# oadrian/GPUFluidSimulator

Measured on AMD Instinct MI355X. Metric: particle-steps/sec, higher is better.
Workload: dtype f32; 1 GPU; dam-break C3: 256x256x256 = 16777216 particles, grid 512^3, box 32.0, dt 5e-7, jittered lattice, FLOWING: timed after 6000 run-up steps on the device (+5 warm-up); particles=16777216, parallelism=1 GPU, whole domain, state=flow, runup_steps=6000

## Files before the change

gpufluidsimulator_amd/capi.py:

```python
from __future__ import annotations

import ctypes as C
import functools
import os

import numpy as np

HERE = os.path.dirname(os.path.abspath(__file__))
LIB_PATH = os.environ.get("SPH_HIP_LIB", os.path.join(HERE, "libsph_hip.so"))

PHASES = ("z-index", "sort", "b-grid", "dens", "force", "collision", "integrate")
HALO_RECORD_FLOATS = 8


class SphError(RuntimeError):
    pass


EXCHANGE_FN = C.CFUNCTYPE(C.c_int, C.c_void_p, C.c_int, C.c_void_p, C.c_size_t, C.c_void_p, C.c_size_t, C.c_void_p, C.c_size_t,
                          C.c_void_p, C.c_size_t, C.c_void_p)


class Transport(C.Structure):
    _fields_ = [("self", C.c_void_p), ("exchange", EXCHANGE_FN), ("host_buffers", C.c_int),
# ... 238 lines not shown
    "sph_get_order": (C.c_int, [_P, _P]),
    "sph_get_cell_range": (C.c_int, [_P, _U32, C.POINTER(_U32), C.POINTER(_U32)]),
    "sph_get_cells": (C.c_int, [_P, _U32, _P, _P, _P]),
    "sph_cell_key": (_U32, [_P, _U32, _U32, _U32]),
    "sph_hash": (C.c_int, [_P]),
    "sph_sort": (C.c_int, [_P]),
    "sph_build_cells": (C.c_int, [_P]),
    "sph_density": (C.c_int, [_P]),
    "sph_force": (C.c_int, [_P]),
    "sph_collide": (C.c_int, [_P]),
    "sph_integrate": (C.c_int, [_P, C.c_float]),
    "sph_step": (C.c_int, [_P, C.c_float, _U32]),
    "sph_step_phased": (C.c_int, [_P, C.c_float, _U32]),
    "sph_force_collide_integrate": (C.c_int, [_P, C.c_float]),
    "sph_timing_enable": (C.c_int, [_P, C.c_int]),
    "sph_timing_get": (C.c_int, [_P, C.POINTER(C.c_float), C.POINTER(_U32)]),
    "sph_timing_reset": (C.c_int, [_P]),
    "sph_last_sort_skipped": (C.c_int, [_P]),
    "sph_sort_stats": (C.c_int, [_P, C.POINTER(C.c_uint64), C.POINTER(C.c_uint64), C.POINTER(C.c_uint64), C.POINTER(C.c_uint32),
                                 C.POINTER(C.c_uint64)]),
    "sph_set_sort_mode": (C.c_int, [_P, C.c_int]),
    "sph_set_direct_hull": (C.c_int, [_P, C.c_uint32]),
    "sph_set_pair_small_launch": (C.c_int, [_P, C.c_uint32]),
    "sph_set_block_order": (C.c_int, [_P, C.c_int, C.c_int, C.c_uint32]),
    "sph_sort_forms": (C.c_int, [_P, C.POINTER(C.c_uint64)]),
    "sph_test_trust_mover_hint": (C.c_int, [_P]),
    "sph_memory_stats": (None, [C.POINTER(C.c_uint64)]),
    "sph_test_fail_alloc": (None, [C.c_uint32]),
    "sph_test_guard": (None, [C.c_uint32, C.c_int]),
    "sph_test_guard_check": (C.c_int, [C.POINTER(C.c_uint64)]),
    "sph_test_scan": (C.c_int, [_P, C.c_int, C.c_uint32, C.c_void_p, C.c_void_p, C.c_void_p]),
    "sph_test_lower_bounds": (C.c_int, [_P, C.c_void_p, C.c_uint32, C.c_void_p, C.c_uint32, C.c_void_p]),
    "sph_set_precision": (C.c_int, [_P, C.c_int]),
    "sph_get_precision": (C.c_int, [_P]),
    "sph_migrants_count": (C.c_int, [_P, C.POINTER(_U32)]),
    "sph_slab_counts": (C.c_int, [_P, C.POINTER(_U32)]),
    "sph_migrants_pack": (C.c_int, [_P, C.POINTER(_P), _U32]),
    "sph_migrants_append": (C.c_int, [_P, _P, _U32]),
    "sph_halo_count": (C.c_int, [_P, C.POINTER(_U32)]),
    "sph_halo_pack": (C.c_int, [_P, C.POINTER(_P), _U32]),
    "sph_halo_pack_counts": (C.c_int, [_P, C.POINTER(_P), _U32, C.POINTER(_U32)]),
    "sph_halo_unpack": (C.c_int, [_P, _P, _U32, _P, _U32]),
    "sph_halo_pack_density": (C.c_int, [_P, C.POINTER(_P), _U32]),
    "sph_halo_unpack_density": (C.c_int, [_P, _P, _P]),
    "sph_layer_histogram": (C.c_int, [_P, _P, _U32]),
    "sph_rccl_unique_id": (C.c_int, [C.c_void_p]),
# ... 668 lines not shown
        return out, total[0]

    def test_lower_bounds(self, keys, targets):
        k, t = np.ascontiguousarray(keys), np.ascontiguousarray(targets)
        assert k.ndim == 1 and t.ndim == 1 and k.dtype == np.uint32 and t.dtype == np.uint32, (k.dtype, t.dtype)
        out = np.empty(t.size, np.uint32)
        _check(self.L.sph_test_lower_bounds(self.h, k.ctypes.data, k.size, t.ctypes.data, t.size, out.ctypes.data))
        return out

    def sort_forms(self):
        out = (C.c_uint64 * 3)()
        _check(self.L.sph_sort_forms(self.h, out))
        return tuple(int(v) for v in out)

    def set_block_order(self, xcd=True, ztile=True, strip_blocks_log2=4):
        _check(self.L.sph_set_block_order(self.h, int(bool(xcd)), int(bool(ztile)), int(strip_blocks_log2)))

    def set_direct_hull(self, slots=512):
        _check(self.L.sph_set_direct_hull(self.h, int(slots) & 0xFFFFFFFF))

    def set_pair_small_launch(self, slots):
        _check(self.L.sph_set_pair_small_launch(self.h, int(slots) & 0xFFFFFFFF))

    def timing_get(self):
        ms = (C.c_float * len(PHASES))()
        steps = _U32(0)
        _check(self.L.sph_timing_get(self.h, ms, C.byref(steps)))
        return {PHASES[k]: float(ms[k]) for k in range(len(PHASES))}, int(steps.value)

    def _pair(self, fn, *a):
        cnt = (_U32 * 2)()
        _check(fn(self.h, cnt, *a))
        return int(cnt[0]), int(cnt[1])

    def slab_counts(self):
        cnt = (_U32 * 4)()
        _check(self.L.sph_slab_counts(self.h, cnt))
        return tuple(int(v) for v in cnt)

    def force_collide_integrate(self, dt): _check(self.L.sph_force_collide_integrate(self.h, float(dt)))

    def migrants_count(self): return self._pair(self.L.sph_migrants_count)
    def halo_count(self): return self._pair(self.L.sph_halo_count)

    def migrants_pack(self, buf_lo, buf_hi, capacity):
        _check(self.L.sph_migrants_pack(self.h, (_P * 2)(buf_lo, buf_hi), int(capacity)))
# ... 26 lines not shown
```

gpufluidsimulator_amd/csrc/sph_capi.hip:

```cpp
#include "sph_device.hpp"

#include <cmath>
#include <cstdarg>
#include <cstdlib>
#include <cstring>
#include <mutex>
#include <new>
#include <vector>

namespace sph {

template <class T>
__global__ __launch_bounds__(1024) void k_test_scan(const T* __restrict__ in, uint32_t n, T* __restrict__ out, T* __restrict__ total) {
    __shared__ T lds[1024 / 64];
    const T sum = scan_array_one_block<1024>(n, lds, [&](uint32_t i) { return in[i]; }, [&](uint32_t i, T before) { out[i] = before; });
    if (threadIdx.x == 0) *total = sum;
}

template <class T>
static int test_scan(sph_ctx* c, Buffers& mem, uint32_t n, const void* in, void* out, void* total) {
    T *d_in = nullptr, *d_out = nullptr, *d_total = nullptr;
    int rc;
    if ((rc = mem.alloc(&d_in, n, false)) || (rc = mem.alloc(&d_out, n, false)) || (rc = mem.alloc(&d_total, 1, false))) return rc;
    if (n) SPH_HIP(hipMemcpyAsync(d_in, in, (size_t)n * sizeof(T), hipMemcpyHostToDevice, c->stream));
// ... 215 lines not shown
    c->device = device;
    c->ghost_layers = slab ? ghost_layers : 1u;
    int rc = derive(c, p, z_lo, z_hi, slab);
    if (rc) { delete c; return rc; }
    c->cap = capacity; c->gcap = gcap; c->tot = capacity + 2 * gcap; c->slab = slab;
    c->own_off = gcap;
    c->pos_out_cap = slab ? 0 : capacity;
    Buffers& m = c->mem;
    const size_t tot = (size_t)c->tot + 256;
    rc = m.alloc(&c->posi, tot, true);
    if (!rc) rc = m.alloc(&c->velr, tot, true);
    if (!rc) rc = m.alloc(&c->posi2, tot, true);
    if (!rc) rc = m.alloc(&c->velr2, tot, true);
    if (!rc) rc = m.alloc(&c->keyS, tot, true);
    if (!rc) rc = m.alloc(&c->keyS2, tot, true);
    if (!rc) rc = m.alloc(&c->dp, tot, true);
    if (!rc) rc = m.alloc(&c->cw, tot, true);
    if (!rc) rc = m.alloc(&c->fpress, tot, false);
    if (!rc) rc = m.alloc(&c->fvisc, tot, false);
    if (!rc) rc = m.alloc(&c->dvel, tot, false);
    if (!rc) rc = m.alloc(&c->pos_out, (size_t)c->pos_out_cap, false);
    if (!rc) rc = m.alloc(&c->table.base, (size_t)c->grid.ncells + 2, true);
    if (!rc) table_init(c, c->table.base, c->grid.ncells);
    if (!rc) rc = sort_buffers_alloc(c);
    if (const char* env = getenv("SPH_BLOCK_ORDER")) {
        int x = 1, z = 1, sh = 4, zd = 1, xr = 1;
        if (sscanf(env, "%d,%d,%d,%d,%d", &x, &z, &sh, &zd, &xr) >= 1) {
            c->order_xcd = x != 0; c->order_ztile = z != 0; if (sh >= 1 && sh <= 10) c->order_strip_sh = (uint32_t)sh;
            c->order_ztile_dens = zd != 0; c->order_xrot = xr != 0;
        }
    }
    if (const char* env = getenv("SPH_PAIR_SMALL_SLOTS")) {
        unsigned long v = 0;
        if (sscanf(env, "%lu", &v) == 1) c->pair_small_slots = v > 0xFFFFFFFFul ? 0xFFFFFFFFu : (uint32_t)v;
    }
    if (const char* env = getenv("SPH_PAIR_CLAMP")) {
        int v = 1;
        if (sscanf(env, "%d", &v) == 1) c->pair_clamp = v != 0;
    }
    if (rc) { m.free_all(); delete c; return rc; }
    *out = c;
    return SPH_OK;
}

void timing_collect(sph_ctx* c) {
    for (size_t k = 0; k + 3 <= c->events.size(); k += 3) {
        hipEvent_t a = c->events[k], b = c->events[k + 1];
        int phase = (int)(intptr_t)c->events[k + 2];
        hipEventSynchronize(b);
        float ms = 0.f;
        if (hipEventElapsedTime(&ms, a, b) == hipSuccess) c->ph_ms[phase] += ms;
        hipEventDestroy(a);
        hipEventDestroy(b);
    }
    c->events.clear();
}

int step_hash(sph_ctx* c, bool ghosts_to_sort) {
    PhaseTimer t(c, SPH_PH_ZINDEX);
    const SlotRange live = live_slots(c);
    int rc = c->sort_merge && c->order_valid && table_covers(c, live.lo, live.hi) ? table_leave_to_sort(c, ghosts_to_sort)
// ... 815 lines not shown
}

int sph_set_block_order(sph_ctx* c, int xcd, int ztile, uint32_t strip_blocks_log2) {
    SPH_REQUIRE(c, SPH_E_INVALID, "null context");
    SPH_REQUIRE(strip_blocks_log2 >= 1u && strip_blocks_log2 <= 10u, SPH_E_INVALID, "strip of 2^%u blocks", strip_blocks_log2);
    c->order_xcd = xcd != 0;
    c->order_ztile = c->order_ztile_dens = ztile != 0;
    c->order_strip_sh = strip_blocks_log2;
    return SPH_OK;
}

int sph_set_direct_hull(sph_ctx* c, uint32_t slots) {
    SPH_REQUIRE(c, SPH_E_INVALID, "null context");
    c->direct_hull = slots;
    return SPH_OK;
}

int sph_set_pair_small_launch(sph_ctx* c, uint32_t slots) {
    SPH_REQUIRE(c, SPH_E_INVALID, "null context");
    c->pair_small_slots = slots;
    return SPH_OK;
}

int sph_sort_stats(sph_ctx* c, uint64_t* sorts, uint64_t* merges, uint64_t* skips, uint32_t* last_movers,
                   uint64_t* movers_total) {
    SPH_REQUIRE(c, SPH_E_INVALID, "null context");
    SPH_HIP(hipSetDevice(c->device));
    SPH_HIP(hipStreamSynchronize(c->stream));
    if (movers_total) {
        unsigned long long t = 0;
        SPH_HIP(hipMemcpy(&t, c->mm_total, sizeof(t), hipMemcpyDeviceToHost));
        *movers_total = t;
    }
    if (sorts) *sorts = c->sort_calls;
    if (merges) *merges = c->sort_merges;
    if (skips) *skips = c->sort_skips;
    if (last_movers) *last_movers = c->mm_count_host[HW_MOVERS];
    return SPH_OK;
}

void sph_memory_stats(uint64_t out[3]) {
    if (out) for (int k = 0; k < 3; k++) out[k] = g_mem_stats[k].load();
}

void sph_test_fail_alloc(uint32_t k) { g_fail_alloc.store(k); }

// ... 35 lines not shown
```

gpufluidsimulator_amd/csrc/sph_common.hpp:

```cpp
#pragma once

#include <hip/hip_runtime.h>

#include <atomic>
#include <cstdint>
#include <cstdio>
#include <cstring>
#include <string>
#include <utility>
#include <vector>

#include "../../include/sph_hip.h"

namespace sph {

constexpr int WAVE = 64;
#ifndef SPH_SORT_KPT
#define SPH_SORT_KPT 16
#endif
constexpr uint32_t SORT_TILE_KEYS = 256 * SPH_SORT_KPT;
#ifndef SPH_PAIR_SMALL_SLOTS_DEFAULT
#define SPH_PAIR_SMALL_SLOTS_DEFAULT 524288u
#endif
constexpr uint32_t MM_TILE_CHUNKS = 256;
// ... 115 lines not shown
        return SPH_OK;
    }
    static void drop(const Rec& r) {
        void* base = r.p;
        if (r.band) { guard_retire(r.p, r.bytes, r.band, r.pinned); base = (char*)r.p - r.band; }
        if (r.pinned) hipHostFree(base); else hipFree(base);
        g_mem_stats[r.pinned] -= r.bytes; g_mem_stats[2] -= 1;
    }
};

enum class TableLeft : uint8_t {
    NOTHING,
    OWNED,
    OWNED_AND_GHOSTS
};

struct CellTable {
    uint2* cells = nullptr;
    uint2* base = nullptr;
    uint32_t alloc = 0;
    uint32_t lo = 0, hi = 0;
    bool valid = false;
    TableLeft left = TableLeft::NOTHING;
};

struct MoverMarks {
    bool marked = false;
    bool scanned = false;
    uint32_t off = 0, n = 0;
    uint32_t scan_seq = 0;
    bool counted_valid = false;
};

enum HostWord : uint32_t {
    HW_MOVERS = 0,
    HW_FIRST_KEY,
    HW_LAST_KEY,
    HW_BUILD_SEQ,
    HW_COUNT_SEQ,
    HW_WORDS = 8
};

struct ObstacleBodyBlock {
    double quat[4];
    float off[3], u[3], pivot[3], omega[3];
    float rot[9], P[3];
};

struct Obstacle {
    sph_obstacle_grid grid{};
    float* phi = nullptr;
    float* brick = nullptr;
    float off[3] = {0.f, 0.f, 0.f}, vel[3] = {0.f, 0.f, 0.f};
    bool posed = false;
    float pivot[3] = {0.f, 0.f, 0.f}, omega[3] = {0.f, 0.f, 0.f};
    double quat[4] = {1.0, 0.0, 0.0, 0.0};
    bool sense = false;
    double* rows = nullptr;
    uint32_t* wmask = nullptr;
    double* load = nullptr;
    bool body = false;
    sph_obstacle_body bd{};
// ... 69 lines not shown
    float* rd_sf_normal = nullptr;
    bool rd_surface = false;
    bool rd_sf_thick_on = false;
    bool rd_solids = false;
    sph_solid_style rd_solid_style{};
    float* rd_so_depth = nullptr;
    uint32_t* rd_so_slot = nullptr;
    float* rd_so_normal = nullptr;

    uint32_t* mesh_field = nullptr;
    uint32_t* mesh_vbase = nullptr;
    uint32_t* mesh_aux = nullptr;
    float* mesh_vpos = nullptr;
    float* mesh_vnrm = nullptr;
    uint32_t* mesh_tri = nullptr;
    uint32_t mesh_nodes_cap = 0, mesh_v_cap = 0, mesh_t_cap = 0;
    uint32_t mesh_dims[3] = {0, 0, 0};
    uint32_t mesh_nv = 0, mesh_nt = 0;
    bool mesh_valid = false;

    uint32_t direct_hull = 512;
    uint32_t pair_small_slots = SPH_PAIR_SMALL_SLOTS_DEFAULT;
    bool pair_clamp = true;
    bool order_xcd = true, order_ztile = true;
    bool order_ztile_dens = true, order_xrot = true;
    uint32_t order_strip_sh = 4;

    sph::CellTable table;
    bool keys_fresh = false;

    uint32_t* k0 = nullptr; uint32_t* v0 = nullptr;
    uint32_t* k1 = nullptr; uint32_t* v1 = nullptr;
    uint32_t* os_hist = nullptr;
    uint32_t* os_base = nullptr;
    uint32_t* os_tickets = nullptr;
    uint32_t* os_tot = nullptr;
    uint32_t os_groups_cap = 0;
    unsigned long long* os_status = nullptr;
    uint32_t* os_status32 = nullptr;
    uint32_t os_epoch = 0;
    uint32_t* os_err_host = nullptr;
    uint32_t* os_err_dev = nullptr;
    uint32_t sort_blocks_cap = 0;
    uint32_t key_bits = 0;
    const uint32_t* last_perm = nullptr;
    bool keep_perm = false;
// ... 163 lines not shown
    return z[b];
}
inline LbTargets layer_bound_targets(const sph_ctx* c) {
    const uint32_t layer = c->grid.g[0] * c->grid.g[1], G = c->ghost_layers, zl = c->grid.zl;
    return LbTargets{{bound_layer(B_OWN_BEGIN, G, zl) * layer, bound_layer(B_FIRST_END, G, zl) * layer,
                      bound_layer(B_LAST_BEGIN, G, zl) * layer, bound_layer(B_OWN_END, G, zl) * layer}, 4u};
}
int launch_headers(hipStream_t st, float4* out_lo, float4* out_hi, float4 lo, float4 hi);
int sort_buffers_alloc(sph_ctx* c);
int tracked_buffers_alloc(sph_ctx* c);

inline uint32_t ceil_div(uint32_t a, uint32_t b) { return (a + b - 1) / b; }

inline void results_stale(sph_ctx* c) { c->have_dens = c->have_force = c->have_coll = false; }
inline void mover_count_unknown(sph_ctx* c) { c->sort_form_both_until = c->sort_calls + 5; }
inline void positions_moved(sph_ctx* c) { c->keys_fresh = false; c->stage = sph_ctx::ST_LOADED; }
inline void order_lost(sph_ctx* c) { positions_moved(c); c->order_valid = false; }
inline void swap_state(sph_ctx* c, bool keys) {
    std::swap(c->posi, c->posi2);
    std::swap(c->velr, c->velr2);
    if (keys) { std::swap(c->keyS, c->keyS2); c->own_off = c->gcap; }
}
inline bool table_covers(const sph_ctx* c, uint32_t lo, uint32_t hi) { return c->table.valid && c->table.lo == lo && c->table.hi == hi; }
inline void table_init(sph_ctx* c, uint2* base, uint32_t alloc) { c->table.base = base; c->table.cells = base + 1; c->table.alloc = alloc; }
inline void table_set(sph_ctx* c, uint32_t lo, uint32_t hi) { c->table.lo = lo; c->table.hi = hi; c->table.valid = true; }
struct SlotRange { uint32_t lo, hi; };
inline SlotRange live_slots(const sph_ctx* c) { return SlotRange{c->own_off - c->n_glo, c->own_off + c->n + c->n_ghi}; }

inline void pack_records(uint32_t n, const float* pos, const float* vel, const uint32_t* index, uint32_t first, float4* hp, float4* hv) {
    for (size_t i = 0; i < n; i++) {
        const uint32_t idx = index ? index[i] : first + (uint32_t)i;
        float w;
        memcpy(&w, &idx, 4);
        hp[i] = make_float4(pos[3 * i], pos[3 * i + 1], pos[3 * i + 2], w);
        hv[i] = vel ? make_float4(vel[3 * i], vel[3 * i + 1], vel[3 * i + 2], 0.f) : make_float4(0.f, 0.f, 0.f, 0.f);
    }
}

struct PhaseTimer {
    sph_ctx* c; int phase; hipEvent_t a = nullptr, b = nullptr;
    PhaseTimer(sph_ctx* c_, int ph) : c(c_), phase(ph) {
        if (!c->timing) return;
        if (hipEventCreate(&a) != hipSuccess || hipEventCreate(&b) != hipSuccess) { a = b = nullptr; return; }
        hipEventRecord(a, c->stream);
    }
    ~PhaseTimer() {
// ... 11 lines not shown
```

gpufluidsimulator_amd/csrc/sph_pairs.hip:

```cpp
#include "sph_device.hpp"

namespace sph {

#ifndef SPH_PAIR_THREADS
#define SPH_PAIR_THREADS 256
#endif
constexpr int PAIR_THREADS = SPH_PAIR_THREADS;
constexpr int PAIR_WAVES = PAIR_THREADS / WAVE;
#ifndef SPH_DENS_THREADS
#define SPH_DENS_THREADS SPH_PAIR_THREADS
#endif
constexpr int DENS_THREADS = SPH_DENS_THREADS;
constexpr int SMALL_THREADS_PAIR = 128;
static inline bool small_blocks(const sph_ctx* c) { return c->n < c->pair_small_slots; }
static inline bool pair_clamp(const sph_ctx* c) { return c->pair_clamp && c->phys.h <= 1.f && c->phys.h2 <= 1.f; }
constexpr int PIECE = 128;

typedef float v2f __attribute__((ext_vector_type(2)));
typedef const volatile __attribute__((address_space(3))) v2f* lds_v2f_ptr;
typedef const volatile __attribute__((address_space(3))) float* lds_f32_ptr;
typedef const volatile __attribute__((address_space(3))) char* lds_byte_ptr;

__global__ __launch_bounds__(256) void k_cells_clear(const uint32_t* __restrict__ key, uint32_t lo, uint32_t hi,
                                                     uint2* __restrict__ cells) {
    uint32_t s = lo + blockIdx.x * 256u + threadIdx.x;
    if (s >= hi) return;
    uint32_t k = key[s];
    if (s == lo || key[s - 1] != k) cells[k] = make_uint2(0u, 0u);
}

__global__ __launch_bounds__(256) void k_cells_build(const uint32_t* __restrict__ key, uint32_t lo, uint32_t hi,
                                                     uint2* __restrict__ cells, volatile uint32_t* __restrict__ ends_host, uint32_t seq) {
    cells_build_thread(key, lo, hi, cells, ends_host, seq, blockIdx.x * 256u + threadIdx.x);
}

__global__ __launch_bounds__(256) void k_cells_clear2(const uint32_t* __restrict__ key, uint32_t lo0, uint32_t hi0,
                                                      uint32_t lo1, uint32_t hi1, uint2* __restrict__ cells) {
    const uint32_t t = blockIdx.x * 256u + threadIdx.x, n0 = hi0 - lo0;
    const uint32_t lo = t < n0 ? lo0 : lo1, hi = t < n0 ? hi0 : hi1;
    const uint32_t s = t < n0 ? lo0 + t : lo1 + (t - n0);
    if (s >= hi) return;
    const uint32_t k = key[s];
    if (s == lo || key[s - 1] != k) cells[k] = make_uint2(0u, 0u);
}

__global__ __launch_bounds__(256) void k_cells_build2(const uint32_t* __restrict__ key, uint32_t lo0, uint32_t hi0,
                                                      uint32_t lo1, uint32_t hi1, uint2* __restrict__ cells) {
    const uint32_t t = blockIdx.x * 256u + threadIdx.x, n0 = hi0 - lo0;
    const uint32_t lo = t < n0 ? lo0 : lo1, hi = t < n0 ? hi0 : hi1;
    const uint32_t s = t < n0 ? lo0 + t : lo1 + (t - n0);
    if (s >= hi) return;
    const uint32_t k = key[s];
    if (s == lo || key[s - 1] != k) cells[k].x = s;
    if (s + 1 == hi || key[s + 1] != k) cells[k].y = s + 1;
}

int launch_cells_clear_2ranges(sph_ctx* c, uint32_t lo0, uint32_t hi0, uint32_t lo1, uint32_t hi1) {
    if (hi0 < lo0) hi0 = lo0;
    if (hi1 < lo1) hi1 = lo1;
    const uint32_t tot = (hi0 - lo0) + (hi1 - lo1);
    if (!tot) return SPH_OK;
    hipLaunchKernelGGL(k_cells_clear2, dim3(ceil_div(tot, 256)), dim3(256), 0, c->stream, c->keyS, lo0, hi0, lo1, hi1, c->table.cells);
    SPH_HIP(hipGetLastError());
    return SPH_OK;
}

int launch_cells_build_2ranges(sph_ctx* c, uint32_t lo0, uint32_t hi0, uint32_t lo1, uint32_t hi1) {
    if (hi0 < lo0) hi0 = lo0;
    if (hi1 < lo1) hi1 = lo1;
    const uint32_t tot = (hi0 - lo0) + (hi1 - lo1);
    if (!tot) return SPH_OK;
    hipLaunchKernelGGL(k_cells_build2, dim3(ceil_div(tot, 256)), dim3(256), 0, c->stream, c->keyS, lo0, hi0, lo1, hi1, c->table.cells);
    SPH_HIP(hipGetLastError());
    return SPH_OK;
}

void table_forget(sph_ctx* c) { c->table.valid = false; c->table.left = TableLeft::NOTHING; }

int launch_cells_clear(sph_ctx* c) {
    const CellTable& t = c->table;
    if (t.valid && t.hi > t.lo) {
        hipLaunchKernelGGL(k_cells_clear, dim3(ceil_div(t.hi - t.lo, 256)), dim3(256), 0, c->stream, c->keyS, t.lo, t.hi, t.cells);
        SPH_HIP(hipGetLastError());
    }
    table_forget(c);
    return SPH_OK;
}

int table_drop_ends(sph_ctx* c, uint32_t m_lo, uint32_t m_hi) {
    const uint32_t lo = c->own_off, hi = c->own_off + c->n;
    if (!table_covers(c, lo, hi)) return SPH_OK;
    const int rc = launch_cells_clear_2ranges(c, lo, lo + m_lo, hi - m_hi, hi);
    if (rc) return rc;
    c->table.lo += m_lo;
    c->table.hi -= m_hi;
    return SPH_OK;
}

int table_drop_ghosts(sph_ctx* c) {
    const uint32_t lo = c->own_off, hi = c->own_off + c->n;
// ... 4 lines not shown

int table_leave_to_sort(sph_ctx* c, bool ghosts_too) {
    if (ghosts_too && (c->n_glo | c->n_ghi)) { c->table.left = TableLeft::OWNED_AND_GHOSTS; return SPH_OK; }
    c->table.left = TableLeft::OWNED;
    return table_drop_ghosts(c);
}

TableLeft table_take_left(sph_ctx* c) {
    const TableLeft left = c->table.valid ? c->table.left : TableLeft::NOTHING;
    c->table.left = TableLeft::NOTHING;
    return left;
}

int launch_cells_clear_range(sph_ctx* c, uint32_t lo, uint32_t hi) {
    if (hi <= lo) return SPH_OK;
    hipLaunchKernelGGL(k_cells_clear, dim3(ceil_div(hi - lo, 256)), dim3(256), 0, c->stream, c->keyS, lo, hi, c->table.cells);
    SPH_HIP(hipGetLastError());
    return SPH_OK;
}

int launch_cells_build_range(sph_ctx* c, uint32_t lo, uint32_t hi, uint32_t seq) {
    if (hi <= lo) return SPH_OK;
    uint32_t* ends = (lo == c->own_off && hi == c->own_off + c->n) ? c->mm_count_host_dev + HW_FIRST_KEY : (uint32_t*)nullptr;
    hipLaunchKernelGGL(k_cells_build, dim3(cells_build_blocks(hi - lo)), dim3(256), 0, c->stream, c->keyS, lo, hi, c->table.cells, ends,
                       ends ? seq : 0u);
    SPH_HIP(hipGetLastError());
    return SPH_OK;
}

int launch_cells_build(sph_ctx* c) {
    const SlotRange live = live_slots(c);
    int rc;
    if (table_covers(c, c->own_off, c->own_off + c->n)) {
        rc = launch_cells_build_2ranges(c, live.lo, c->own_off, c->own_off + c->n, live.hi);
    } else {
        rc = launch_cells_clear(c);
        if (!rc) rc = launch_cells_build_range(c, live.lo, live.hi);
    }
    if (rc) return rc;
    table_set(c, live.lo, live.hi);
    return SPH_OK;
}

struct Rows {
    uint32_t lo[9], hi[9];
};

__device__ __forceinline__ void lane_rows(const uint2* __restrict__ cells, const GridDesc& g, uint32_t key, bool active,
// ... 89 lines not shown
constexpr int UNROLL = SPH_DENS_UNROLL;
#ifndef SPH_FORCE_UNROLL
#define SPH_FORCE_UNROLL 2
#endif
#ifndef SPH_EXACT_DIV
#define SPH_EXACT_DIV 0
#endif

struct Hulls {
    uint32_t A[9], B[9];
};

__device__ __forceinline__ void wave_hulls(const Rows& R, Hulls& H) {
#pragma unroll
    for (int r = 0; r < 9; r++) {
        const uint64_t m = __ballot(R.hi[r] > R.lo[r]);
        if (m == 0ull) { H.A[r] = 0u; H.B[r] = 0u; continue; }
        const int first = __builtin_ctzll(m), last = 63 - __builtin_clzll(m);
        H.A[r] = (uint32_t)__builtin_amdgcn_readlane((int)R.lo[r], first);
        H.B[r] = (uint32_t)__builtin_amdgcn_readlane((int)R.hi[r], last);
    }
}

template <class Load, class Store, class Work>
__device__ __forceinline__ void traverse(const Hulls& H, Load&& load, Store&& store, Work&& work) {
    auto first_behind = [&](int r, uint32_t& a) {
        bool any = false;
#pragma unroll
        for (int q = 8; q > r; q--) {
            uint32_t end = H.B[q];
            asm volatile("" : "+s"(end));
            if (end != 0u) { a = H.A[q]; any = true; }
        }
        return any;
    };
    uint32_t a_next = 0u;
    if (!first_behind(-1, a_next)) return;
    load(a_next);
#pragma unroll
    for (int r = 0; r < 9; r++) {
        if (H.A[r] >= H.B[r]) continue;
        for (uint32_t a = H.A[r]; a < H.B[r]; a += PIECE) {
            store();
            bool more = true;
            a_next = a + PIECE;
            if (a_next >= H.B[r]) more = first_behind(r, a_next);
            if (more) load(a_next);
            wave_lds_sync();
            work(r, a, min(a + PIECE, H.B[r]));
            wave_lds_sync();
        }
    }
}

__device__ __forceinline__ bool wave_has_long_hull(const Hulls& H, uint32_t key, uint32_t direct_hull) {
    const uint32_t k0 = (uint32_t)__builtin_amdgcn_readlane((int)key, 0), k1 = (uint32_t)__builtin_amdgcn_readlane((int)key, 63);
    if (k1 - k0 <= 64u && direct_hull >= 128u) return false;
    bool any = false;
#pragma unroll
    for (int r = 0; r < 9; r++) any = any || (H.B[r] > H.A[r] && H.B[r] - H.A[r] > direct_hull);
    return any;
}

template <class Row>
__device__ __forceinline__ void direct_rows(const uint2* __restrict__ cells, const GridDesc& g, uint32_t key, bool active,
                                            Row&& row) {
#pragma clang loop unroll(disable)
    for (int r = 0; r < 9; r++) {
        uint32_t l0, l1;
        lane_row_one(cells, g, key, active, r / 3 - 1, r % 3 - 1, l0, l1);
        const uint32_t len = l1 > l0 ? l1 - l0 : 0u;
        const uint32_t T = wave_max_u32(len);
// ... 123 lines not shown
            const uint32_t len = l1 > l0 ? l1 - l0 : 0u;
            const uint32_t rel = len ? l0 - a : 0u;
            uint32_t idx = slice + rel;
            const uint32_t tmin = wave_min_u32_uniform_first(len) & ~(uint32_t)(UNROLL - 1);
            lds_v2f_ptr zp = (lds_v2f_ptr)(((rel & 1u) ? (const float*)s_zo - 1 : (const float*)s_z) + idx);
            auto group = [&](uint32_t t, bool check) {
#pragma unroll
                for (int u = 0; u < UNROLL; u += 2) {
                    const v2f xy0 = ((lds_v2f_ptr)s_xy)[idx + u], xy1 = ((lds_v2f_ptr)s_xy)[idx + u + 1];
                    const v2f zz = zp[u >> 1];
                    pair_math(xy0.x, xy0.y, zz.x, !check || t + u < len);
                    pair_math(xy1.x, xy1.y, zz.y, !check || t + u + 1 < len);
                }
                idx += UNROLL;
                zp += UNROLL / 2;
            };
            uint32_t t = 0;
            for (; t < tmin; t += UNROLL) group(t, false);
#ifdef SPH_PAIR_STATS
            const uint32_t stat_t0 = t;
#endif
            for (; __ballot(t < len) != 0ull; t += UNROLL) group(t, true);
            PAIR_STAT(11, t - stat_t0);
        });
    finish();
}

typedef _Float16 h2 __attribute__((ext_vector_type(2)));
typedef const volatile __attribute__((address_space(3))) h2* lds_h2_ptr;
typedef _Float16 h4 __attribute__((ext_vector_type(4)));
typedef const volatile __attribute__((address_space(3))) h4* lds_h4_ptr;

__device__ __forceinline__ h2 h2_splat(float x) { const _Float16 v = (_Float16)x; return h2{v, v}; }
__device__ __forceinline__ h2 h2_mask(bool lo, bool hi) {
    const uint32_t bits = (lo ? 0x3C00u : 0u) | (hi ? 0x3C000000u : 0u);
    return __builtin_bit_cast(h2, bits);
}

constexpr int HPAIRS = PIECE / 2;
constexpr int LDS_PAIRS = (PAIR_WAVES + 1) * HPAIRS + 8;
constexpr int HUNROLL = 4;

struct PairWalk {
    uint32_t idx;
    uint32_t whole;
    bool odd;
// ... 793 lines not shown
    return force_finish(c, integrate, mark, dt);
}

static int launch_density_targets(sph_ctx* c, const Targets& tg, uint32_t threads) {
    if (threads == 0) return SPH_OK;
    if (c->precision == SPH_PRECISION_MIXED_F16)
        hipLaunchKernelGGL(k_density_h, dim3(ceil_div(threads, PAIR_THREADS)), dim3(PAIR_THREADS), 0, c->stream, c->posi,
                           c->keyS, c->table.cells, c->dp, c->cw, tg, c->grid, c->phys);
    else {
#define SPH_LAUNCH_DENSITY_T(T, CL)                                                                                             \
    hipLaunchKernelGGL((k_density<T, CL>), dim3(ceil_div(threads, (uint32_t)T)), dim3(T), 0, c->stream, c->posi, c->keyS,        \
                       c->table.cells, c->dp, c->cw, tg, c->grid, c->phys)
        if (pair_clamp(c)) {
            if (small_blocks(c)) SPH_LAUNCH_DENSITY_T(SMALL_THREADS_PAIR, true); else SPH_LAUNCH_DENSITY_T(DENS_THREADS, true);
        } else {
            if (small_blocks(c)) SPH_LAUNCH_DENSITY_T(SMALL_THREADS_PAIR, false); else SPH_LAUNCH_DENSITY_T(DENS_THREADS, false);
        }
#undef SPH_LAUNCH_DENSITY_T
    }
    SPH_HIP(hipGetLastError());
    return SPH_OK;
}

int launch_density_hole(sph_ctx* c, uint32_t lo, uint32_t hi, uint32_t hole_lo, uint32_t hole_hi) {
    if (hi <= lo) return SPH_OK;
    uint32_t threads;
    Targets tg = targets_with_hole(lo, hi, hole_lo, hole_hi, threads);
    tg.direct_hull = c->direct_hull;
    const uint32_t bt = c->precision == SPH_PRECISION_MIXED_F16 ? (uint32_t)PAIR_THREADS : (small_blocks(c) ? (uint32_t)SMALL_THREADS_PAIR : (uint32_t)DENS_THREADS);
    tg.order = block_order(c, ceil_div(threads, bt), c->order_ztile_dens);
    return launch_density_targets(c, tg, threads);
}

int launch_density_range(sph_ctx* c, uint32_t lo, uint32_t hi) { return launch_density_hole(c, lo, hi, hi, hi); }

int launch_density_dev_range(sph_ctx* c, const uint32_t* range_dev, uint32_t max_count) {
    const Targets tg{0u, 0u, 0xFFFFFFFFu, 0u, range_dev, c->direct_hull, BlockOrder{0u, 0u, 0u, 0u, 0u}};
    return launch_density_targets(c, tg, max_count);
}

template <class... Sph>
__global__ __launch_bounds__(256) void k_integrate(float4* __restrict__ posi, float4* __restrict__ velr,
                                                   const float2* __restrict__ dp, const float4* __restrict__ fpress,
                                                   const float4* __restrict__ fvisc, const float4* __restrict__ dvel,
                                                   float4* __restrict__ pos_by_index, uint32_t lo, uint32_t hi, float dt,
                                                   Phys ph, Sph... sp) {
    uint32_t i = lo + blockIdx.x * 256u + threadIdx.x;
    if (i >= hi) return;
    float4 pi = posi[i], vi = velr[i];
    const float4 fp = fpress[i], fv = fvisc[i], dv = dvel[i];
    integrate_one(ph, dt, pi, vi, dp[i].x, fp.x + fv.x, fp.y + fv.y, fp.z + fv.z, dv.x, dv.y, dv.z, at_slot(sp, i - lo)...);
// ... 25 lines not shown
```

include/sph_hip.h:

```cpp
#ifndef SPH_HIP_H
#define SPH_HIP_H

#include <stddef.h>
#include <stdint.h>

#ifdef __cplusplus
extern "C" {
#endif

#define SPH_ABI_VERSION 2

enum {
    SPH_OK = 0,
    SPH_E_INVALID = -1,
    SPH_E_DEVICE = -2,
    SPH_E_NOMEM = -3,
    SPH_E_CAPACITY = -4,
    SPH_E_STATE = -5,
    SPH_E_PEER = -6
};

typedef struct sph_ctx sph_ctx;

typedef struct sph_params {
// ... 230 lines not shown
 int sph_get_cells(sph_ctx* c, uint32_t max_cells, uint32_t* key, uint32_t* start, uint32_t* count);
 uint32_t sph_cell_key(const sph_ctx* c, uint32_t x, uint32_t y, uint32_t z);

int sph_hash(sph_ctx* c);
int sph_sort(sph_ctx* c);
int sph_build_cells(sph_ctx* c);
int sph_density(sph_ctx* c);
int sph_force(sph_ctx* c);
int sph_collide(sph_ctx* c);
int sph_integrate(sph_ctx* c, float dt);
int sph_step(sph_ctx* c, float dt, uint32_t n_steps);
int sph_step_phased(sph_ctx* c, float dt, uint32_t n_steps);
int sph_force_collide_integrate(sph_ctx* c, float dt);

int sph_timing_enable(sph_ctx* c, int on);
int sph_timing_get(sph_ctx* c, float ms[SPH_PH_COUNT], uint32_t* n_steps);
int sph_timing_reset(sph_ctx* c);
 int sph_sort_stats(sph_ctx* c, uint64_t* sorts, uint64_t* merges, uint64_t* skips, uint32_t* last_movers,
                   uint64_t* movers_total);
 int sph_sort_forms(const sph_ctx* c, uint64_t out[3]);
 int sph_set_sort_mode(sph_ctx* c, int merge);
 int sph_set_direct_hull(sph_ctx* c, uint32_t slots);
 int sph_set_pair_small_launch(sph_ctx* c, uint32_t slots);
 int sph_set_block_order(sph_ctx* c, int xcd, int ztile, uint32_t strip_blocks_log2);
 int sph_last_sort_skipped(const sph_ctx* c);

#define SPH_HALO_RECORD_FLOATS 8
int sph_migrants_count(sph_ctx* c, uint32_t count[2]);
int sph_slab_counts(sph_ctx* c, uint32_t count[4]);
int sph_migrants_pack(sph_ctx* c, void* buf_dev[2], uint32_t capacity);
int sph_migrants_append(sph_ctx* c, const void* buf_dev, uint32_t n);
int sph_halo_count(sph_ctx* c, uint32_t count[2]);
int sph_halo_pack(sph_ctx* c, void* buf_dev[2], uint32_t capacity);
int sph_halo_pack_counts(sph_ctx* c, void* buf_dev[2], uint32_t capacity, const uint32_t count[2]);
int sph_halo_unpack(sph_ctx* c, const void* lo_dev, uint32_t n_lo, const void* hi_dev, uint32_t n_hi);
int sph_halo_pack_density(sph_ctx* c, void* buf_dev[2], uint32_t capacity);
int sph_halo_unpack_density(sph_ctx* c, const void* lo_dev, const void* hi_dev);
int sph_layer_histogram(sph_ctx* c, uint32_t* hist, uint32_t n_layers);

enum { SPH_TAG_MIGRANTS = 1, SPH_TAG_HALO_A = 2, SPH_TAG_HALO_B = 3, SPH_TAG_MIGRANTS_REST = 4, SPH_TAG_PING = 5,
       SPH_TAG_RECUT_COUNTS = 6, SPH_TAG_RECUT = 7,
       SPH_TAG_ONE = 8,
       SPH_TAG_ONE_REST = 9 };
typedef struct sph_transport {
    void* self;
    int (*exchange)(void* self, int tag, const void* send_lo, size_t send_lo_bytes, void* recv_lo, size_t recv_lo_bytes,
// ... 68 lines not shown
```

Measured before the change: 4.293 billion particle-steps/s.

## Compute density for same-cell particle pairs per thread using item list

```diff
diff --git a/gpufluidsimulator_amd/capi.py b/gpufluidsimulator_amd/capi.py
--- a/gpufluidsimulator_amd/capi.py
+++ b/gpufluidsimulator_amd/capi.py
@@ -284,6 +284,8 @@
     "sph_set_sort_mode": (C.c_int, [_P, C.c_int]),
     "sph_set_direct_hull": (C.c_int, [_P, C.c_uint32]),
     "sph_set_pair_small_launch": (C.c_int, [_P, C.c_uint32]),
+    "sph_set_density_pairs": (C.c_int, [_P, C.c_int]),
+    "sph_get_items": (C.c_int, [_P, C.c_uint32, _P]),
     "sph_set_block_order": (C.c_int, [_P, C.c_int, C.c_int, C.c_uint32]),
     "sph_sort_forms": (C.c_int, [_P, C.POINTER(C.c_uint64)]),
     "sph_test_trust_mover_hint": (C.c_int, [_P]),
@@ -998,6 +1000,14 @@
     def set_pair_small_launch(self, slots):
         _check(self.L.sph_set_pair_small_launch(self.h, int(slots) & 0xFFFFFFFF))
 
+    def set_density_pairs(self, on=True):
+        _check(self.L.sph_set_density_pairs(self.h, 1 if on else 0))
+
+    def items(self):
+        out = np.empty(max(self.n, 1), dtype=np.uint32)
+        m = _check(self.L.sph_get_items(self.h, out.size, out.ctypes.data))
+        return out[:m].copy()
+
     def timing_get(self):
         ms = (C.c_float * len(PHASES))()
         steps = _U32(0)
diff --git a/gpufluidsimulator_amd/csrc/sph_capi.hip b/gpufluidsimulator_amd/csrc/sph_capi.hip
--- a/gpufluidsimulator_amd/csrc/sph_capi.hip
+++ b/gpufluidsimulator_amd/csrc/sph_capi.hip
@@ -261,6 +261,13 @@
     if (!rc) rc = m.alloc(&c->pos_out, (size_t)c->pos_out_cap, false);
     if (!rc) rc = m.alloc(&c->table.base, (size_t)c->grid.ncells + 2, true);
     if (!rc) table_init(c, c->table.base, c->grid.ncells);
+    if (!slab) {
+        const size_t nb = cells_build_blocks(capacity) + 1;
+        if (!rc) rc = m.alloc(&c->item_slot, (size_t)capacity, false);
+        if (!rc) rc = m.alloc(&c->item_mask, nb * 4 * CELLS_SPT, false);
+        if (!rc) rc = m.alloc(&c->item_blk, nb, false);
+        if (!rc) rc = m.alloc(&c->item_count, 1, false);
+    }
     if (!rc) rc = sort_buffers_alloc(c);
     if (const char* env = getenv("SPH_BLOCK_ORDER")) {
         int x = 1, z = 1, sh = 4, zd = 1, xr = 1;
@@ -276,6 +283,10 @@
     if (const char* env = getenv("SPH_PAIR_CLAMP")) {
         int v = 1;
         if (sscanf(env, "%d", &v) == 1) c->pair_clamp = v != 0;
+    }
+    if (const char* env = getenv("SPH_DENSITY_PAIRS")) {
+        int v = 1;
+        if (sscanf(env, "%d", &v) == 1) c->density_pairs = v != 0;
     }
     if (rc) { m.free_all(); delete c; return rc; }
     *out = c;
@@ -1137,6 +1148,27 @@
     return SPH_OK;
 }
 
+int sph_set_density_pairs(sph_ctx* c, int on) {
+    SPH_REQUIRE(c, SPH_E_INVALID, "null context");
+    c->density_pairs = on != 0;
+    return SPH_OK;
+}
+
+int sph_get_items(sph_ctx* c, uint32_t max_items, uint32_t* item_slot) {
+    SPH_REQUIRE(c, SPH_E_INVALID, "null context");
+    SPH_HIP(hipSetDevice(c->device));
+    SPH_HIP(hipStreamSynchronize(c->stream));
+    if (!items_live(c, c->own_off, c->own_off + c->n)) return 0;
+    uint32_t count = 0;
+    SPH_HIP(hipMemcpy(&count, c->item_count, sizeof(count), hipMemcpyDeviceToHost));
+    const uint32_t m = count < max_items ? count : max_items;
+    if (m && item_slot) {
+        SPH_HIP(hipMemcpy(item_slot, c->item_slot, (size_t)m * sizeof(uint32_t), hipMemcpyDeviceToHost));
+        for (uint32_t t = 0; t < m; t++) item_slot[t] -= c->own_off;
+    }
+    return (int)count;
+}
+
 int sph_sort_stats(sph_ctx* c, uint64_t* sorts, uint64_t* merges, uint64_t* skips, uint32_t* last_movers,
                    uint64_t* movers_total) {
     SPH_REQUIRE(c, SPH_E_INVALID, "null context");
diff --git a/gpufluidsimulator_amd/csrc/sph_common.hpp b/gpufluidsimulator_amd/csrc/sph_common.hpp
--- a/gpufluidsimulator_amd/csrc/sph_common.hpp
+++ b/gpufluidsimulator_amd/csrc/sph_common.hpp
@@ -161,6 +161,8 @@
     uint32_t lo = 0, hi = 0;
     bool valid = false;
     TableLeft left = TableLeft::NOTHING;
+    bool items = false;
+    uint32_t items_lo = 0, items_hi = 0;
 };
 
 struct MoverMarks {
@@ -177,6 +179,7 @@
     HW_LAST_KEY,
     HW_BUILD_SEQ,
     HW_COUNT_SEQ,
+    HW_ITEMS,
     HW_WORDS = 8
 };
 
@@ -292,6 +295,9 @@
     uint32_t direct_hull = 512;
     uint32_t pair_small_slots = SPH_PAIR_SMALL_SLOTS_DEFAULT;
     bool pair_clamp = true;
+    bool density_pairs = true;
+    uint32_t* item_slot = nullptr; uint32_t* item_count = nullptr; uint32_t* item_blk = nullptr;
+    unsigned long long* item_mask = nullptr;
     bool order_xcd = true, order_ztile = true;
     bool order_ztile_dens = true, order_xrot = true;
     uint32_t order_strip_sh = 4;
@@ -501,6 +507,9 @@
     if (keys) { std::swap(c->keyS, c->keyS2); c->own_off = c->gcap; }
 }
 inline bool table_covers(const sph_ctx* c, uint32_t lo, uint32_t hi) { return c->table.valid && c->table.lo == lo && c->table.hi == hi; }
+inline bool items_live(const sph_ctx* c, uint32_t lo, uint32_t hi) {
+    return c->table.items && c->table.items_lo == lo && c->table.items_hi == hi && table_covers(c, lo, hi);
+}
 inline void table_init(sph_ctx* c, uint2* base, uint32_t alloc) { c->table.base = base; c->table.cells = base + 1; c->table.alloc = alloc; }
 inline void table_set(sph_ctx* c, uint32_t lo, uint32_t hi) { c->table.lo = lo; c->table.hi = hi; c->table.valid = true; }
 struct SlotRange { uint32_t lo, hi; };
diff --git a/gpufluidsimulator_amd/csrc/sph_pairs.hip b/gpufluidsimulator_amd/csrc/sph_pairs.hip
--- a/gpufluidsimulator_amd/csrc/sph_pairs.hip
+++ b/gpufluidsimulator_amd/csrc/sph_pairs.hip
@@ -15,6 +15,10 @@
 static inline bool small_blocks(const sph_ctx* c) { return c->n < c->pair_small_slots; }
 static inline bool pair_clamp(const sph_ctx* c) { return c->pair_clamp && c->phys.h <= 1.f && c->phys.h2 <= 1.f; }
 constexpr int PIECE = 128;
+constexpr int PIECE2 = 256;
+static inline bool items_wanted(const sph_ctx* c) {
+    return c->density_pairs && c->item_slot && c->precision == SPH_PRECISION_F32 && !small_blocks(c) && DENS_THREADS == 256;
+}
 
 typedef float v2f __attribute__((ext_vector_type(2)));
 typedef const volatile __attribute__((address_space(3))) v2f* lds_v2f_ptr;
@@ -32,6 +36,116 @@
 __global__ __launch_bounds__(256) void k_cells_build(const uint32_t* __restrict__ key, uint32_t lo, uint32_t hi,
                                                      uint2* __restrict__ cells, volatile uint32_t* __restrict__ ends_host, uint32_t seq) {
     cells_build_thread(key, lo, hi, cells, ends_host, seq, blockIdx.x * 256u + threadIdx.x);
+}
+
+__global__ __launch_bounds__(256) void k_cells_build_items(const uint32_t* __restrict__ key, uint32_t lo, uint32_t hi,
+                                                           uint2* __restrict__ cells, volatile uint32_t* __restrict__ ends_host,
+                                                           uint32_t seq, unsigned long long* __restrict__ item_mask,
+                                                           uint32_t* __restrict__ item_blk) {
+    __shared__ uint32_t s_cnt[4];
+    const uint32_t t = blockIdx.x * 256u + threadIdx.x, lane = threadIdx.x & 63u, wave = threadIdx.x >> 6;
+    cells_build_thread(key, lo, hi, cells, ends_host, seq, t);
+    const uint32_t s0 = lo + t * CELLS_SPT;
+    const bool in = s0 < hi;
+    const uint32_t w0 = (uint32_t)__builtin_amdgcn_readfirstlane((int)(lo + (blockIdx.x * 256u + wave * 64u) * CELLS_SPT));
+    constexpr uint32_t BACK = 16;
+    uint32_t kb[BACK + 1] = {};
+    const bool w_in = w0 > lo && w0 < hi;
+    if (w_in) {
+#pragma unroll
+        for (uint32_t i = 0; i <= BACK; i++) kb[i] = key[w0 >= lo + i ? w0 - i : lo];
+    }
+    uint32_t kk[CELLS_SPT + 1] = {};
+    uint32_t last = 0u;
+    if (in) {
+        kk[1] = key[s0];
+        kk[0] = s0 > lo ? key[s0 - 1] : ~kk[1];
+#pragma unroll
+        for (uint32_t j = 1; j < CELLS_SPT; j++) kk[j + 1] = s0 + j < hi ? key[s0 + j] : ~kk[j];
+#pragma unroll
+        for (uint32_t j = 0; j < CELLS_SPT; j++) if (kk[j] != kk[j + 1]) last = s0 + j + 1u;
+    }
+    uint32_t wave_start = 0u;
+    if (w_in) {
+        uint32_t run = 0u;
+        bool same = true;
+#pragma unroll
+        for (uint32_t i = 1; i <= BACK; i++) {
+            same = same && w0 >= lo + i && kb[i] == kb[0];
+            run += same ? 1u : 0u;
+        }
+        uint32_t b = w0 - run;
+        if (run == BACK) b = first_not(lo, b, [&](uint32_t i) { return key[i] < kb[0]; });
+        wave_start = b + 1u;
+    }
+    const unsigned long long has = __ballot(last != 0u) & ((1ull << lane) - 1ull);
+    uint32_t start = (uint32_t)__shfl((int)last, has ? 63 - __builtin_clzll(has) : 0, 64);
+    if (has == 0ull) start = wave_start;
+    uint32_t bits = 0u;
+#pragma unroll
+    for (uint32_t j = 0; j < CELLS_SPT; j++) {
+        const uint32_t s = s0 + j;
+        if (in && s < hi) {
+            if (kk[j] != kk[j + 1]) start = s + 1u;
+            if (((s + 1u - start) & 1u) == 0u) bits |= 1u << j;
+        }
+    }
+    unsigned long long mj[CELLS_SPT];
+    uint32_t cnt = 0u;
+#pragma unroll
+    for (uint32_t j = 0; j < CELLS_SPT; j++) {
+        mj[j] = __ballot((bits >> j) & 1u);
+        cnt += (uint32_t)__builtin_popcountll(mj[j]);
+    }
+    if (lane < CELLS_SPT)
+        item_mask[(size_t)(blockIdx.x * 4u + wave) * CELLS_SPT + lane] = lane == 0u ? mj[0] : lane == 1u ? mj[1] : lane == 2u ? mj[2] : mj[3];
+    if (lane == 0u) s_cnt[wave] = cnt;
+    __syncthreads();
+    if (threadIdx.x == 0u) item_blk[blockIdx.x] = s_cnt[0] + s_cnt[1] + s_cnt[2] + s_cnt[3];
+}
+
+constexpr uint32_t ITEMS_SCAN_THREADS = 1024, ITEMS_SCAN_PER = 16;
+__global__ __launch_bounds__(ITEMS_SCAN_THREADS) void k_items_scan(uint32_t* __restrict__ item_blk, uint32_t nb,
+                                                                   uint32_t* __restrict__ item_count) {
+    __shared__ uint32_t lds[ITEMS_SCAN_THREADS / 64];
+    uint32_t carry = 0u;
+    for (uint32_t base = 0; base < nb; base += ITEMS_SCAN_THREADS * ITEMS_SCAN_PER) {
+        const uint32_t i0 = base + threadIdx.x * ITEMS_SCAN_PER;
+        uint32_t v[ITEMS_SCAN_PER], sum = 0u;
+#pragma unroll
+        for (uint32_t q = 0; q < ITEMS_SCAN_PER; q++) v[q] = i0 + q < nb ? item_blk[i0 + q] : 0u;
+#pragma unroll
+        for (uint32_t q = 0; q < ITEMS_SCAN_PER; q++) { const uint32_t x = v[q]; v[q] = sum; sum += x; }
+        uint32_t total;
+        const uint32_t before = carry + block_scan_excl<ITEMS_SCAN_THREADS / 64>(sum, lds, total);
+#pragma unroll
+        for (uint32_t q = 0; q < ITEMS_SCAN_PER; q++) if (i0 + q < nb) item_blk[i0 + q] = before + v[q];
+        carry += total;
+    }
+    if (threadIdx.x == 0u) item_count[0] = carry;
+}
+
+__global__ __launch_bounds__(256) void k_items_write(const unsigned long long* __restrict__ item_mask,
+                                                     const uint32_t* __restrict__ item_blk, uint32_t lo,
+                                                     uint32_t* __restrict__ item_slot, const uint32_t* __restrict__ item_count,
+                                                     volatile uint32_t* __restrict__ items_host) {
+    if (blockIdx.x == 0u && threadIdx.x == 0u) *items_host = item_count[0];
+    const uint32_t lane = threadIdx.x & 63u;
+    const uint32_t wave = (uint32_t)__builtin_amdgcn_readfirstlane((int)(threadIdx.x >> 6));
+    const unsigned long long* const mb = item_mask + (size_t)blockIdx.x * (4u * CELLS_SPT);
+    uint32_t off = item_blk[blockIdx.x];
+    for (uint32_t q = 0; q < wave * CELLS_SPT; q++) off += (uint32_t)__builtin_popcountll(mb[q]);
+    const unsigned long long below = (1ull << lane) - 1ull;
+    unsigned long long mj[CELLS_SPT];
+#pragma unroll
+    for (uint32_t j = 0; j < CELLS_SPT; j++) {
+        mj[j] = mb[wave * CELLS_SPT + j];
+        off += (uint32_t)__builtin_popcountll(mj[j] & below);
+    }
+    const uint32_t s0 = lo + (blockIdx.x * 256u + threadIdx.x) * CELLS_SPT;
+#pragma unroll
+    for (uint32_t j = 0; j < CELLS_SPT; j++)
+        if ((mj[j] >> lane) & 1ull) item_slot[off++] = s0 + j;
 }
 
 __global__ __launch_bounds__(256) void k_cells_clear2(const uint32_t* __restrict__ key, uint32_t lo0, uint32_t hi0,
@@ -75,7 +189,7 @@
     return SPH_OK;
 }
 
-void table_forget(sph_ctx* c) { c->table.valid = false; c->table.left = TableLeft::NOTHING; }
+void table_forget(sph_ctx* c) { c->table.valid = false; c->table.left = TableLeft::NOTHING; c->table.items = false; }
 
 int launch_cells_clear(sph_ctx* c) {
     const CellTable& t = c->table;
@@ -126,8 +240,18 @@
 int launch_cells_build_range(sph_ctx* c, uint32_t lo, uint32_t hi, uint32_t seq) {
     if (hi <= lo) return SPH_OK;
     uint32_t* ends = (lo == c->own_off && hi == c->own_off + c->n) ? c->mm_count_host_dev + HW_FIRST_KEY : (uint32_t*)nullptr;
-    hipLaunchKernelGGL(k_cells_build, dim3(cells_build_blocks(hi - lo)), dim3(256), 0, c->stream, c->keyS, lo, hi, c->table.cells, ends,
-                       ends ? seq : 0u);
+    const uint32_t nb = cells_build_blocks(hi - lo);
+    if (ends && items_wanted(c)) {
+        hipLaunchKernelGGL(k_cells_build_items, dim3(nb), dim3(256), 0, c->stream, c->keyS, lo, hi, c->table.cells, ends, seq,
+                           c->item_mask, c->item_blk);
+        hipLaunchKernelGGL(k_items_scan, dim3(1), dim3(ITEMS_SCAN_THREADS), 0, c->stream, c->item_blk, nb, c->item_count);
+        hipLaunchKernelGGL(k_items_write, dim3(nb), dim3(256), 0, c->stream, c->item_mask, c->item_blk, lo, c->item_slot,
+                           c->item_count, c->mm_count_host_dev + HW_ITEMS);
+        SPH_HIP(hipGetLastError());
+        c->table.items = true; c->table.items_lo = lo; c->table.items_hi = hi;
+        return SPH_OK;
+    }
+    hipLaunchKernelGGL(k_cells_build, dim3(nb), dim3(256), 0, c->stream, c->keyS, lo, hi, c->table.cells, ends, ends ? seq : 0u);
     SPH_HIP(hipGetLastError());
     return SPH_OK;
 }
@@ -263,7 +387,7 @@
     }
 }
 
-template <class Load, class Store, class Work>
+template <int P = PIECE, class Load, class Store, class Work>
 __device__ __forceinline__ void traverse(const Hulls& H, Load&& load, Store&& store, Work&& work) {
     auto first_behind = [&](int r, uint32_t& a) {
         bool any = false;
@@ -281,14 +405,14 @@
 #pragma unroll
     for (int r = 0; r < 9; r++) {
         if (H.A[r] >= H.B[r]) continue;
-        for (uint32_t a = H.A[r]; a < H.B[r]; a += PIECE) {
+        for (uint32_t a = H.A[r]; a < H.B[r]; a += (uint32_t)P) {
             store();
             bool more = true;
-            a_next = a + PIECE;
+            a_next = a + (uint32_t)P;
             if (a_next >= H.B[r]) more = first_behind(r, a_next);
             if (more) load(a_next);
             wave_lds_sync();
-            work(r, a, min(a + PIECE, H.B[r]));
+            work(r, a, min(a + (uint32_t)P, H.B[r]));
             wave_lds_sync();
         }
     }
@@ -458,6 +582,142 @@
 #endif
             for (; __ballot(t < len) != 0ull; t += UNROLL) group(t, true);
             PAIR_STAT(11, t - stat_t0);
+        });
+    finish();
+}
+
+#ifndef SPH_DENS2_OCC
+#define SPH_DENS2_OCC 5
+#endif
+constexpr int DENS2_THREADS = 256;
+template <bool CLAMP>
+__global__ __launch_bounds__(DENS2_THREADS, SPH_DENS2_OCC) void k_density2(const float4* __restrict__ posi,
+                                                                           const uint32_t* __restrict__ keyS,
+                                                                           const uint2* __restrict__ cells,
+                                                                           float2* __restrict__ dp, float2* __restrict__ cw,
+                                                                           const uint32_t* __restrict__ item_slot,
+                                                                           const uint32_t* __restrict__ item_count,
+                                                                           Targets tg, GridDesc g, Phys ph) {
+    constexpr int ENT = (DENS2_THREADS / WAVE + 1) * PIECE2 + 8;
+    __shared__ float2 s_xy[ENT];
+    __shared__ __attribute__((aligned(8))) float s_z[ENT];
+    __shared__ __attribute__((aligned(8))) float s_zo_[ENT + 2];
+    float* const s_zo = s_zo_ + 2;
+    const uint32_t n_items = item_count[0];
+    const uint32_t nb = (n_items + (uint32_t)DENS2_THREADS - 1u) / (uint32_t)DENS2_THREADS;
+    if (blockIdx.x >= nb) return;
+    BlockOrder order = tg.order;
+    if ((nb >> 3) < (1u << (order.lb_sh + order.nl_sh))) order.nl_sh = 0u;
+    const uint32_t rot = max(nb >> 6, 1u);
+    const uint32_t block = ordered_block(blockIdx.x < rot ? nb - rot + blockIdx.x : blockIdx.x - rot, nb, order);
+    for (uint32_t k = threadIdx.x; k < ENT; k += DENS2_THREADS) {
+        s_xy[k] = make_float2(0.f, 0.f);
+        s_z[k] = 0.f;
+        s_zo_[k] = 0.f;
+        if (k < 2u) s_zo_[ENT + k] = 0.f;
+    }
+    __syncthreads();
+    const uint32_t wave = threadIdx.x >> 6, lane = threadIdx.x & 63u;
+    const uint32_t slice = wave * PIECE2;
+    const uint32_t first = (block * (uint32_t)(DENS2_THREADS / WAVE) + wave) * WAVE;
+    if (first >= n_items) return;
+    const bool active = first + lane < n_items;
+    const uint32_t ia = item_slot[active ? first + lane : n_items - 1u];
+    const uint32_t my_key = keyS[ia];
+    const bool two = ia + 1u < tg.hi && keyS[ia + 1u] == my_key;
+    const uint32_t ib = two ? ia + 1u : ia;
+    const float4 pa = posi[ia], pb = posi[ib];
+    Rows R;
+    lane_rows(cells, g, my_key, active, R);
+    Hulls H;
+    wave_hulls(R, H);
+    float4 q0, q1, q2, q3;
+    const uint32_t lane16 = lane << 4;
+    float acc_a = 0.f, acc_b = 0.f;
+    const float h2_v = in_vgpr(ph.h2);
+    auto pair_math = [&](float x, float y, float z, bool valid) {
+        const float ax = pa.x - x, ay = pa.y - y, az = pa.z - z;
+        const float bx = pb.x - x, by = pb.y - y, bz = pb.z - z;
+        float da = cut_below_zero<CLAMP>(fmaf(-az, az, fmaf(-ay, ay, fmaf(-ax, ax, h2_v))));
+        float db = cut_below_zero<CLAMP>(fmaf(-bz, bz, fmaf(-by, by, fmaf(-bx, bx, h2_v))));
+        da = valid ? da : 0.f;
+        db = valid ? db : 0.f;
+        acc_a = fmaf(da * da, da, acc_a);
+        acc_b = fmaf(db * db, db, acc_b);
+    };
+    auto finish = [&]() {
+        if (active) {
+            const float rho = acc_a * ph.poly6_mass;
+            const float p = fmaxf(0.f, ph.gas_constant * (rho - ph.rest_density));
+            dp[ia] = make_float2(rho, p);
+            cw[ia] = neighbour_terms(ph, rho, p);
+            if (two) {
+                const float rho_b = acc_b * ph.poly6_mass;
+                const float p_b = fmaxf(0.f, ph.gas_constant * (rho_b - ph.rest_density));
+                dp[ib] = make_float2(rho_b, p_b);
+                cw[ib] = neighbour_terms(ph, rho_b, p_b);
+            }
+        }
+    };
+    if (wave_has_long_hull(H, my_key, tg.direct_hull)) {
+        const uint32_t me = item_slot[active ? first + lane : n_items - 1u];
+        direct_rows(cells, g, keyS[me], active, [&](uint32_t l0, uint32_t len, uint32_t T) {
+            for (uint32_t t = 0; t < T; t += 2u) {
+                float4 q[2];
+#pragma unroll
+                for (uint32_t u = 0; u < 2u; u++) q[u] = posi[t + u < len ? l0 + t + u : me];
+#pragma unroll
+                for (uint32_t u = 0; u < 2u; u++) pair_math(q[u].x, q[u].y, q[u].z, t + u < len);
+            }
+        });
+        finish();
+        return;
+    }
+    traverse<PIECE2>(
+        H,
+        [&](uint32_t a) {
+            const float4* const p = posi + a;
+            q0 = lane_elem(p, lane16);
+            q1 = lane_elem(p + WAVE, lane16);
+            q2 = lane_elem(p + 2 * WAVE, lane16);
+            q3 = lane_elem(p + 3 * WAVE, lane16);
+        },
+        [&]() {
+            const uint32_t e = slice + lane;
+            s_xy[e] = make_float2(q0.x, q0.y);
+            s_z[e] = q0.z;
+            s_xy[e + WAVE] = make_float2(q1.x, q1.y);
+            s_z[e + WAVE] = q1.z;
+            s_xy[e + 2 * WAVE] = make_float2(q2.x, q2.y);
+            s_z[e + 2 * WAVE] = q2.z;
+            s_xy[e + 3 * WAVE] = make_float2(q3.x, q3.y);
+            s_z[e + 3 * WAVE] = q3.z;
+            s_zo[(int)e - 1] = q0.z;
+            s_zo[e + WAVE - 1u] = q1.z;
+            s_zo[e + 2 * WAVE - 1u] = q2.z;
+            s_zo[e + 3 * WAVE - 1u] = q3.z;
+        },
+        [&](int r, uint32_t a, uint32_t b) {
+            const uint32_t l0 = max(R.lo[r], a), l1 = min(R.hi[r], b);
+            const uint32_t len = l1 > l0 ? l1 - l0 : 0u;
+            const uint32_t rel = len ? l0 - a : 0u;
+            uint32_t idx = slice + rel;
+            const uint32_t tmin = wave_min_u32_uniform_first(len) & ~(uint32_t)(UNROLL - 1);
+            lds_v2f_ptr zp = (lds_v2f_ptr)(((rel & 1u) ? (const float*)s_zo - 1 : (const float*)s_z) + idx);
+            auto group = [&](uint32_t t, bool check) {
+#pragma unroll
+                for (int u = 0; u < UNROLL; u += 2) {
+                    const v2f xy0 = ((lds_v2f_ptr)s_xy)[idx + u], xy1 = ((lds_v2f_ptr)s_xy)[idx + u + 1];
+                    const v2f zz = zp[u >> 1];
+                    pair_math(xy0.x, xy0.y, zz.x, !check || t + u < len);
+                    pair_math(xy1.x, xy1.y, zz.y, !check || t + u + 1 < len);
+                }
+                idx += UNROLL;
+                zp += UNROLL / 2;
+            };
+            uint32_t t = 0;
+            for (; t < tmin; t += UNROLL) group(t, false);
+            for (; __ballot(t < len) != 0ull; t += UNROLL) group(t, true);
         });
     finish();
 }
@@ -1297,11 +1557,25 @@
     return SPH_OK;
 }
 
+static int launch_density_items(sph_ctx* c, Targets tg) {
+    const uint32_t n = tg.hi - tg.lo, hint = c->mm_count_host[HW_ITEMS];
+    const uint32_t items = hint >= (n + 1u) / 2u && hint <= n ? hint : n / 2u + n / 32u;
+    tg.order = block_order(c, ceil_div(items, (uint32_t)DENS2_THREADS), c->order_ztile_dens);
+#define SPH_LAUNCH_DENSITY2(CL)                                                                                                 \
+    hipLaunchKernelGGL((k_density2<CL>), dim3(ceil_div(n, (uint32_t)DENS2_THREADS)), dim3(DENS2_THREADS), 0, c->stream, c->posi, \
+                       c->keyS, c->table.cells, c->dp, c->cw, c->item_slot, c->item_count, tg, c->grid, c->phys)
+    if (pair_clamp(c)) SPH_LAUNCH_DENSITY2(true); else SPH_LAUNCH_DENSITY2(false);
+#undef SPH_LAUNCH_DENSITY2
+    SPH_HIP(hipGetLastError());
+    return SPH_OK;
+}
+
 int launch_density_hole(sph_ctx* c, uint32_t lo, uint32_t hi, uint32_t hole_lo, uint32_t hole_hi) {
     if (hi <= lo) return SPH_OK;
     uint32_t threads;
     Targets tg = targets_with_hole(lo, hi, hole_lo, hole_hi, threads);
     tg.direct_hull = c->direct_hull;
+    if (tg.gap_len == 0u && items_wanted(c) && items_live(c, lo, hi)) return launch_density_items(c, tg);
     const uint32_t bt = c->precision == SPH_PRECISION_MIXED_F16 ? (uint32_t)PAIR_THREADS : (small_blocks(c) ? (uint32_t)SMALL_THREADS_PAIR : (uint32_t)DENS_THREADS);
     tg.order = block_order(c, ceil_div(threads, bt), c->order_ztile_dens);
     return launch_density_targets(c, tg, threads);
diff --git a/include/sph_hip.h b/include/sph_hip.h
--- a/include/sph_hip.h
+++ b/include/sph_hip.h
@@ -276,6 +276,8 @@
  int sph_set_sort_mode(sph_ctx* c, int merge);
  int sph_set_direct_hull(sph_ctx* c, uint32_t slots);
  int sph_set_pair_small_launch(sph_ctx* c, uint32_t slots);
+ int sph_set_density_pairs(sph_ctx* c, int on);
+ int sph_get_items(sph_ctx* c, uint32_t max_items, uint32_t* item_slot);
  int sph_set_block_order(sph_ctx* c, int xcd, int ztile, uint32_t strip_blocks_log2);
  int sph_last_sort_skipped(const sph_ctx* c);
 
```

Result: faster. 4.350 billion particle-steps/s, median of 6 (+1.3%).
